# ushasigh/srsran-edgeric-5g

Hardware: AMD Instinct MI355X
Metric: pdsch_slots_per_sec (higher is better)
Workload: dtype u32 bit-packed GF(2) + bf16 grid + f32 IQ

## Files before the change

### srsran-edgeric-5g_amd/build.py

```python
import os
import subprocess
import sys

HERE = os.path.dirname(os.path.abspath(__file__))
ROOT = os.path.dirname(HERE)
CSRC = os.path.join(HERE, "csrc")
LIB = os.path.join(CSRC, "libmi355nrphy.so")
SOURCES = ["nrphy_host.cpp", "pdsch_plan_build.cpp", "pdsch_host.cpp", "dl_control_host.cpp", "pdsch_async.cpp", "dl_slot_async.cpp",
           "ofdm_host.cpp", "lower_phy_host.cpp", "demod_host.cpp", "ldpc_dematcher_host.cpp", "ldpc_decoder_host.cpp", "pusch_decoder_host.cpp",
           "csi_rs_host.cpp", "pdsch_kernels.hip", "ofdm_kernels.hip", "ldpc_decoder.hip",
           "ldpc_dematcher.hip", "pusch_decoder.hip", "csi_rs_kernels.hip", "dl_control_kernels.hip", "lower_phy_kernels.hip", "demod_kernels.hip",
           "pusch_demod_host.cpp", "pusch_demod_kernels.hip", "pusch_chest_host.cpp", "pusch_chest_kernels.hip",
           "prach_host.cpp", "prach_kernels.hip", "prach_demod_host.cpp", "prach_demod_kernels.hip", "pucch_host.cpp", "pucch_kernels.hip",
           "pucch2_host.cpp", "pucch2_kernels.hip", "srs_host.cpp", "srs_kernels.hip",
           "uci_host.cpp", "uci_kernels.hip", "ulsch_host.cpp", "ulsch_kernels.hip", "ofh_ul_host.cpp", "ofh_ul_kernels.hip",
           "ofh_dl_host.cpp", "ofh_dl_kernels.hip", "ofh_rx_host.cpp", "ofh_rx_kernels.hip"]
HEADERS = ["nrphy_internal.h", "nrphy_host_internal.h", "pdsch_plan.h", "pdsch_staging_host.h", "ldpc_receive_host.h", "ldpc_base_graph_host.h", "pusch_alloc_host.h", "ulsch_placement_host.h", "nrphy_trace.h", "bits_device.h", "crc24b_fold.h", "ofh_compress_device.h", "ofh_ul_chunk_device.h", "chest_device.h", "chest_host.h", "demod_device.h", "equalize_device.h", "ldpc_device.h", "fft_device.h", "nr_ldpc_bg.inc", "nr_polar_tables.inc", "prach_tables.inc", "prach_demod_tables.inc", "pucch_tables.inc", "srs_tables.inc", "uci_tables.inc",
           os.path.join(ROOT, "include", "mi355_nrphy.h")]
HIPCC = os.environ.get("HIPCC", "/opt/rocm/bin/hipcc")
MAX_COMPILERS = 16
CONTRACT = {}
FLAGS = ["--offload-arch=gfx950", "-O3", "-std=c++17", "-fPIC", "-Wall",
         "-I" + os.path.join(ROOT, "include"), "-I" + CSRC]


def _stale():
    if not os.path.exists(LIB):
        return True
    t = os.path.getmtime(LIB)
    deps = [os.path.join(CSRC, s) for s in SOURCES] + [h if os.path.isabs(h) else os.path.join(CSRC, h) for h in HEADERS]
    return any(os.path.getmtime(d) > t for d in deps)


def build(force=False, verbose=False):
    if not force and not _stale():
        return LIB
    objs = []
    cmds = []
    for src in SOURCES:
        obj = os.path.join(CSRC, os.path.splitext(src)[0] + ".o")
        cmds.append([HIPCC] + FLAGS + [CONTRACT.get(src, "-ffp-contract=off"), "-x", "hip", "-c", os.path.join(CSRC, src),
                     "-o", obj])
        objs.append(obj)
    procs = []
    try:
        while cmds or procs:
            while cmds and len(procs) < MAX_COMPILERS:
                cmd = cmds.pop(0)
                if verbose:
                    print(" ".join(cmd))
                procs.append((cmd, subprocess.Popen(cmd, stdout=subprocess.PIPE, stderr=subprocess.STDOUT)))
            cmd, p = procs.pop(0)
            out, _ = p.communicate(timeout=1800)
            if p.returncode != 0:
                raise RuntimeError("hipcc failed: %s\n%s" % (" ".join(cmd), out.decode(errors="replace")))
            if verbose and out:
                print(out.decode(errors="replace"))
    finally:
        for _, p in procs:
            p.kill()
    cmd = [HIPCC, "--offload-arch=gfx950", "-shared", "-fPIC", "-o", LIB] + objs
    subprocess.run(cmd, check=True, timeout=600)
    return LIB


if __name__ == "__main__":
    print(build(force="--force" in sys.argv, verbose=True))
```

### srsran-edgeric-5g_amd/csrc/nrphy_internal.h

```cpp
#pragma once

#include "mi355_nrphy.h"

#include <hip/hip_runtime.h>
#include <stdint.h>

namespace nrphy {

constexpr int NOF_LIFTING_SIZES = 51;
constexpr int NOF_GRAPHS        = 2 * NOF_LIFTING_SIZES;
constexpr int MAX_BG_ROWS       = 46;
constexpr int MAX_BG_EDGES      = 316;

struct LiftedGraph {
  uint16_t row_ptr[MAX_BG_ROWS + 2];
  uint16_t core_b;
  uint16_t core_s0;
  uint16_t core_s3;
  uint16_t core_mid;
  uint32_t edge[MAX_BG_EDGES];
};

#define NR_POLAR_SUBBLOCK_PATTERN                                                                                       \
  {0, 1, 2, 4, 3, 5, 6, 7, 8, 16, 9, 17, 10, 18, 11, 19, 12, 20, 13, 21, 14, 22, 15, 23, 24, 25, 26, 28, 27, 29, 30, 31}

constexpr int GOLD_JUMP_BITS  = 24;
constexpr int GOLD_X1_WORDS   = 1 << 16;

constexpr uint32_t SCR_PARTS = 4;

constexpr int CRC_POW_WORDS = 288;

struct GoldTables {
  uint32_t x2_jump[GOLD_JUMP_BITS][32];
  uint32_t x2_head[32][32];
  uint32_t crc24b_pow32[CRC_POW_WORDS];
  uint32_t crc24b_table[256];
  uint32_t crc24b_mul[CRC_POW_WORDS][6][16];
  float2 qam_lut[4][256];
};

constexpr int RE_CHUNK = 512;
#define NRPHY_CB_U_GRAPH_OFFSET (2 * 22 * 12 + 80)

enum SymKind : uint32_t { SYM_NONE = 0, SYM_CONTIGUOUS = 1, SYM_TABLE = 2 };

struct PduDev {
  uint64_t tb_offset;
  uint64_t cw_bit_offset;
  uint32_t tb_bytes;
  uint32_t grid_index;
  uint32_t graph;
  uint32_t zc;
  uint32_t kb;
  uint32_t K;
  uint32_t info_bits;
  uint32_t filler;
  uint32_t tb_crc_bits;
  uint32_t cb_crc_bits;
  uint32_t zero_pad;
  uint32_t C;
  uint32_t n_short;
  uint32_t e_short;
  uint32_t e_long;
  uint32_t n_cb;
  uint32_t k0;
  uint32_t nof_rows;
  uint32_t qm;
  uint32_t nof_layers;
  uint32_t nof_ports;
  uint32_t c_init;
  uint32_t item_first;
  uint32_t seed_first;
  uint32_t scr_words;
  uint32_t scr_word_offset;
  uint32_t nof_re;
  uint32_t weights_offset;
  uint32_t dmrs_weights_offset;
  uint32_t nof_prg;
  uint32_t prg_size_subc;
  uint32_t sym_re_start[NRPHY_NSYMB + 1];
  uint32_t sym_kind[NRPHY_NSYMB];
  uint32_t sym_arg[NRPHY_NSYMB];
  uint32_t dmrs_symbol_mask;
  uint32_t dmrs_zero_other_group;
  uint32_t dmrs_c_init[NRPHY_NSYMB];
  uint32_t dmrs_ref_rb;
  uint32_t dmrs_seq_offset;
  uint32_t dmrs_seq_words;
  float    dmrs_amplitude;
  uint32_t prb_mask[2 * NRPHY_PRB_WORDS];
  uint32_t first_prb;
  uint32_t end_prb;
  uint32_t crc_first;
  uint32_t crc_count;
};

struct CbWork {
  uint32_t pdu;
  uint32_t cb;
  uint32_t re_begin;
  uint32_t re_count;
};

constexpr int DMRS_PRB_CHUNK = 32;
#ifndef NRPHY_CRC_WORDS_PER_THREAD
#define NRPHY_CRC_WORDS_PER_THREAD 16
#endif
constexpr uint32_t TB_CRC_REGION_WORDS = 256 * NRPHY_CRC_WORDS_PER_THREAD;
constexpr uint32_t TB_CRC_REGION_BYTES = 4 * TB_CRC_REGION_WORDS;

struct TbCrcTables {
  uint32_t y32[2][4][256];
  uint32_t y1k[2][4][256];
  uint32_t y8k[2][4][256];
  uint32_t yz[2][4][256];
  uint32_t lane[2][64];
};

// ... 622 lines not shown
```

### srsran-edgeric-5g_amd/csrc/pdsch_kernels.hip

```cpp
#include "ldpc_device.h"

#ifndef NRPHY_PHASE_A_STAGED
#define NRPHY_PHASE_A_STAGED 1
#endif

#ifdef NRPHY_PROBES
#define NRPHY_STAGE(p) ((p).profile_stage)
#else
#define NRPHY_STAGE(p) 0u
#endif

namespace nrphy {

__global__ __launch_bounds__(TB_CRC_THREADS) void prologue_kernel(PdschLaunch p, const uint8_t* __restrict__ d_tb)
{
  constexpr uint32_t LDS_WORDS = TB_CRC_LDS_WORDS;
  __shared__ __attribute__((aligned(16))) uint32_t lds[LDS_WORDS];
  static_assert(LDS_WORDS >= GOLD_RING_WORDS, "LDS of the sequence role");
  const uint32_t tid = threadIdx.x;

  uint32_t scr_index = blockIdx.x, crc_index = blockIdx.x - p.n_scr_work;
  bool     scr_role  = blockIdx.x < p.n_scr_work;
  if (p.prologue_order == 1 && p.n_scr_work != 0 && p.n_crc_work != 0) {
    const uint32_t total = p.n_scr_work + p.n_crc_work;
    const uint32_t xcd = blockIdx.x & 7u, turn = blockIdx.x >> 3, q = total >> 3, r = total & 7u;
    const uint32_t pos = xcd * q + (xcd < r ? xcd : r) + turn;
    const uint32_t s0 = (uint32_t)(((uint64_t)pos * p.n_scr_work + total - 1u) / total);
    const uint32_t s1 = (uint32_t)(((uint64_t)(pos + 1u) * p.n_scr_work + total - 1u) / total);
    scr_role  = s1 > s0;
    scr_index = s0;
    crc_index = pos - s0;
  }
  NRPHY_WG_TRACE_MARK(0);
  NRPHY_WG_TRACE_WHERE(scr_role ? 1 : 2);
  if (scr_role) {
    if (NRPHY_STAGE(p) == 8) {
      return;
    }
    const auto*    swc   = to_constant(&p.scr_work[scr_index]);
    const uint32_t first = swc->first, count = swc->count;
    const bool     with_dmrs = swc->with_dmrs != 0;
    PduRef         pd    = *to_constant(&p.pdus[swc->pdu]);
    const uint32_t wave = tid / WAVE, lane = tid % WAVE;
    constexpr uint32_t DMRS_WAVES = TB_CRC_THREADS / WAVE - 1, DMRS_SCRATCH = (GOLD_RING_WORDS - 2048u) / DMRS_WAVES;
    static_assert(GOLD_SEED_WORDS <= 2048u && GOLD_RING_WORDS > 2048u, "LDS of the sequence role");
    static_assert((12u * NRPHY_MAX_RB + 31u) / 32u + 1u <= DMRS_SCRATCH, "DM-RS scratch per wave");
    if (wave == 0) {
      if (count == 0) {
        return;
      }
      if (p.scr_as_words != 0) {
        constexpr uint32_t SCR_STORE_ROWS = 8;
        uint32_t*       out = p.scr_seq + pd.scr_word_offset + first;
        const uint32_t* x1  = p.x1_words + first;
        gold_sequence_blocks_wave(p.gold, pd.c_init, first, count, lds, lane, [&](uint32_t base, uint32_t avail) {
          for (uint32_t k0 = lane; k0 < avail; k0 += SCR_STORE_ROWS * WAVE) {
            uint32_t x[SCR_STORE_ROWS];
// ... 230 lines not shown
    const uint32_t pad = (32u - (n & 31u)) & 31u;
    const uint32_t nw  = (n + pad) >> 5;
    const uint32_t per = (nw + WAVE - 1) / WAVE;
    uint32_t       a   = lane * per;
    uint32_t       b   = a + per;
    a                  = a > nw ? nw : a;
    b                  = b > nw ? nw : b;
    constexpr uint32_t CRC_MAX_PER = (22u * 384u / 32u + WAVE - 1u) / WAVE;
    const uint32_t     first = b - per, skip = a - first;
    uint32_t           word[CRC_MAX_PER];
    if (pad == 0) {
#pragma unroll
      for (uint32_t i = 0; i != CRC_MAX_PER; ++i) {
        word[i] = 0;
        if (i < per && i >= skip) {
          word[i] = sh->lin[first + i];
        }
      }
    } else {
#pragma unroll
      for (uint32_t i = 0; i != CRC_MAX_PER; ++i) {
        const uint32_t j = first + i;
        word[i]          = 0;
        if (i < per && i >= skip) {
          word[i] = (j == 0) ? sh->lin[0] >> pad : ext32(sh->lin, 32u * j - pad);
        }
      }
    }
    uint32_t res = 0, parity = 0;
#pragma unroll
    for (uint32_t i = 0; i != CRC_MAX_PER; ++i) {
      if (i < per) {
        res = crc24b_fold_word(res, word[i]);
        parity ^= word[i];
      }
    }
    const uint32_t reg = crc24b_fold_finish(res, parity);
    uint32_t part = 0;
    {
      const uint32_t m = nw - b;
#pragma unroll
      for (uint32_t k = 0; k != 6; ++k) {
        part ^= tables->crc24b_mul[m][k][(reg >> (4u * k)) & 15u];
      }
    }
    uint32_t crc = wave_xor(part);
    if (lane == 0) {
      or_bits_lds_exclusive(sh->lin, n, crc << 8, 24);
    }
    wave_sync();
  }
}

struct RmIndex {
  uint32_t fs;
  uint32_t flen;
  uint32_t n_valid;
  uint32_t rank0;
  float    inv_valid;
};

__device__ __forceinline__ RmIndex rm_index_init(PduRef pd)
{
  RmIndex  r;
  uint32_t nsys = (pd.kb - 2u) * pd.zc;
  uint32_t fs   = nsys - pd.filler;
  uint32_t fe   = nsys;
  fs            = fs > pd.n_cb ? pd.n_cb : fs;
  fe            = fe > pd.n_cb ? pd.n_cb : fe;
  r.fs          = fs;
  r.flen        = fe - fs;
  r.n_valid     = pd.n_cb - r.flen;
  r.rank0       = pd.k0 < fs ? pd.k0 : (pd.k0 < fe ? fs : pd.k0 - r.flen);
  r.inv_valid   = 1.0f / (float)r.n_valid;
  return r;
}

template <bool WRAP>
__device__ __forceinline__ uint32_t rm_gather32(const RmIndex& r, const uint32_t* lin, uint32_t zc2, uint32_t t)
{
  uint32_t u = r.rank0 + t;
  if (WRAP && u >= r.n_valid) {
    uint32_t q = (uint32_t)((float)u * r.inv_valid);
    u -= q * r.n_valid;
    if ((int32_t)u < 0) {
      u += r.n_valid;
    } else if (u >= r.n_valid) {
      u -= r.n_valid;
    }
  }
  uint32_t run = (u < r.fs) ? r.fs - u : r.n_valid - u;
  uint32_t out = ext32(lin, (u < r.fs ? u : u + r.flen) + zc2);
  if (run >= 32u) {
    return out;
  }
  out &= topmask(run);
  uint32_t filled = run;
  while (filled < 32u) {
    u += run;
    if (u >= r.n_valid) {
      if (!WRAP) {
        break;
      }
      u = 0;
    }
    run            = (u < r.fs) ? r.fs - u : r.n_valid - u;
    run            = run > 32u - filled ? 32u - filled : run;
    uint32_t piece = ext32(lin, (u < r.fs ? u : u + r.flen) + zc2);
    out |= (piece & topmask(run)) >> filled;
    filled += run;
  }
  return out;
}

__device__ __forceinline__ uint32_t bit_select(uint32_t m, uint32_t a, uint32_t b)
{
  return __builtin_amdgcn_bitop3_b32(m, a, b, 0xCA);
}

__device__ __forceinline__ void transpose8x8(uint32_t& hi, uint32_t& lo)
{
  hi = bit_select(0xAA55AA55u, hi, bit_select(0x55005500u, hi << 7, hi >> 7));
  lo = bit_select(0xAA55AA55u, lo, bit_select(0x55005500u, lo << 7, lo >> 7));
  hi = bit_select(0xCCCC3333u, hi, bit_select(0x33330000u, hi << 14, hi >> 14));
  lo = bit_select(0xCCCC3333u, lo, bit_select(0x33330000u, lo << 14, lo >> 14));
  const uint32_t nhi = bit_select(0xF0F0F0F0u, hi, lo >> 4);
  const uint32_t nlo = bit_select(0x0F0F0F0Fu, lo, hi << 4);
  hi                 = nhi;
  lo                 = nlo;
}

__device__ __forceinline__ void cmul_ref(float xr, float xi, float wr, float wi, float& outr, float& outi)
{
  float t0 = __fmul_rn(xi, wi);
  float t1 = __fmul_rn(xr, wi);
  outr     = __fmaf_rn(xr, wr, -t0);
  outi     = __fmaf_rn(xi, wr, t1);
}

typedef float cf2 __attribute__((ext_vector_type(2)));
__device__ __forceinline__ cf2 cmul_ref_packed(cf2 x, cf2 w)
{
  cf2 t, r;
  asm("v_pk_mul_f32 %0, %1, %2 op_sel:[1,1] op_sel_hi:[0,1]" : "=v"(t) : "v"(x), "v"(w));
  asm("v_pk_fma_f32 %0, %1, %2, %3 op_sel_hi:[1,0,1] neg_lo:[0,0,1]" : "=v"(r) : "v"(x), "v"(w), "v"(t));
  return r;
}
__device__ __forceinline__ cf2 cmul_ref_packed_uniform(cf2 x, cf2 w)
{
  cf2 t, r;
  asm("v_pk_mul_f32 %0, %1, %2 op_sel:[1,1] op_sel_hi:[0,1]" : "=v"(t) : "v"(x), "s"(w));
  asm("v_pk_fma_f32 %0, %1, %2, %3 op_sel_hi:[1,0,1] neg_lo:[0,0,1]" : "=v"(r) : "v"(x), "s"(w), "v"(t));
  return r;
}

typedef __bf16 bf16x2_t __attribute__((ext_vector_type(2)));
typedef float  f32x2_t __attribute__((ext_vector_type(2)));
__device__ __forceinline__ uint32_t pack_cbf16(float re, float im)
{
  f32x2_t  v = {re, im};
  bf16x2_t b = __builtin_convertvector(v, bf16x2_t);
  return *reinterpret_cast<uint32_t*>(&b);
}

__device__ __forceinline__ void grid_store(uint32_t* p, uint32_t v)
{
  __builtin_nontemporal_store(v, p);
}

#ifndef NRPHY_GRID_STORE_AUX
#define NRPHY_GRID_STORE_AUX 2
#endif
#ifndef NRPHY_GRID_BUFFER_STORES
#define NRPHY_GRID_BUFFER_STORES 1
#endif

struct ChunkGeom {
  uint32_t E;
  uint32_t cw_cb;
  uint32_t bit0;
};

template <int QM, int L, bool WRAP>
__device__ __forceinline__ void phase_a(const PdschLaunch& p, PduRef pd, const CbWork& wk, const CbShared& sh,
                                        uint32_t E, uint32_t lane)
{
  const uint32_t esym = E / QM;
  const uint32_t zc2  = 2u * pd.zc;
  const RmIndex  rm   = rm_index_init(pd);
  const uint32_t s0   = wk.re_begin * L;
  const uint32_t nblk = (wk.re_count * L + 31u) >> 5;
  constexpr uint32_t LUT_TRIPS = ((1u << QM) + WAVE - 1u) / WAVE;
  float2             lut[LUT_TRIPS];
#pragma unroll
  for (uint32_t k = 0; k != LUT_TRIPS; ++k) {
    lut[k] = lane + WAVE * k < (1u << QM) ? p.gold->qam_lut[QM / 2 - 1][lane + WAVE * k] : make_float2(0.f, 0.f);
  }
#if NRPHY_PHASE_A_STAGED
  for (uint32_t item = lane; item < QM * nblk; item += WAVE) {
    const uint32_t blk = item / QM, j = item - blk * QM;
    sh.symb[8u * blk + j] = rm_gather32<WRAP>(rm, sh.lin, zc2, j * esym + s0 + 32u * blk);
  }
  wave_sync();
  const uint8_t* rows = reinterpret_cast<const uint8_t*>(sh.symb);
  for (uint32_t item = lane; item < 4u * nblk; item += WAVE) {
    const uint32_t blk = item >> 2, m = item & 3u;
    const uint8_t* b   = rows + 32u * blk + (3u - m);
    uint32_t       r8[8];
#pragma unroll
    for (int j = 0; j != 8; ++j) {
      r8[j] = (j < QM) ? b[4 * j] : 0u;
    }
    uint32_t hi = (r8[0] << 24) | (r8[1] << 16) | (r8[2] << 8) | r8[3];
    uint32_t lo = (r8[4] << 24) | (r8[5] << 16) | (r8[6] << 8) | r8[7];
    transpose8x8(hi, lo);
    sh.symb[8u * blk + 2u * m]      = hi;
    sh.symb[8u * blk + 2u * m + 1u] = lo;
  }
#else
  for (uint32_t blk = lane; blk < nblk; blk += WAVE) {
    uint32_t row[8];
#pragma unroll
    for (int j = 0; j != 8; ++j) {
      row[j] = (j < QM) ? rm_gather32<WRAP>(rm, sh.lin, zc2, (uint32_t)j * esym + s0 + 32u * blk) : 0u;
    }
#pragma unroll
    for (int m = 0; m != 4; ++m) {
      const int sft = 24 - 8 * m;
      uint32_t  hi  = (((row[0] >> sft) & 0xFFu) << 24) | (((row[1] >> sft) & 0xFFu) << 16) |
                    (((row[2] >> sft) & 0xFFu) << 8) | ((row[3] >> sft) & 0xFFu);
      uint32_t lo = (((row[4] >> sft) & 0xFFu) << 24) | (((row[5] >> sft) & 0xFFu) << 16) |
                    (((row[6] >> sft) & 0xFFu) << 8) | ((row[7] >> sft) & 0xFFu);
      transpose8x8(hi, lo);
      sh.symb[8u * blk + 2u * m]      = hi;
      sh.symb[8u * blk + 2u * m + 1u] = lo;
    }
  }
#endif
  if (lane < 8) {
    sh.symb[8u * nblk + lane] = 0;
  }
#pragma unroll
  for (uint32_t k = 0; k != LUT_TRIPS; ++k) {
    if (lane + WAVE * k < (1u << QM)) {
      reinterpret_cast<float2*>(sh.u)[lane + WAVE * k] = lut[k];
    }
  }
  wave_sync();
}

__device__ __forceinline__ void pin_scalar(cf2& w)
{
  asm volatile("" : "+s"(w));
}

struct ChunkMap {
  uint32_t re0;
  uint32_t word0;
  bool     aligned;
  const uint32_t* gwords;
};

template <int QM, int L>
__device__ __forceinline__ uint32_t global_bits(const ChunkGeom& g, const ChunkMap& cm, uint32_t re_count, uint32_t r)
{
  uint32_t bits = 0;
  if (r < re_count) {
    if (QM * L == 32 && cm.aligned) {
      bits = (cm.gwords + cm.word0)[r];
    } else {
      bits = ext32(cm.gwords, g.bit0 + r * (uint32_t)(QM * L));
    }
  }
  return bits;
}
template <int QM, int L>
__device__ __forceinline__ uint32_t x2_bits(const uint32_t* x2, const ChunkGeom& g, const ChunkMap& cm, uint32_t r)
{
  if (QM * L == 32 && cm.aligned) {
    return x2[r];
  }
  return ext32(x2, (g.bit0 & 31u) + r * (uint32_t)(QM * L));
}

template <int QM, int L, bool WORDS>
__device__ __forceinline__ void re_bits(const CbShared& sh, const ChunkGeom& g, const ChunkMap& cm,
                                        uint32_t re_count, uint32_t r, uint32_t& bytes, uint32_t& gbits)
{
  if constexpr (L == 4) {
    bytes = sh.symb[r];
  } else {
// ... 150 lines not shown
      for (int l = 0; l != L; ++l) {
        const uint32_t raw = ((bytes >> (24 - 8 * l)) & 0xFFu) >> (8 - QM);
        v_rm |= raw << (32 - (l + 1) * QM);
      }
      if (d_cw_rm) {
        or_bits_global(d_cw_rm, cw_bit0 + (uint64_t)r * LQ, v_rm, LQ);
      }
      if (d_cw_scr) {
        or_bits_global(d_cw_scr, cw_bit0 + (uint64_t)r * LQ, v_rm ^ (gbits & topmask(LQ)), LQ);
      }
    }
  }
  if (d_grid == nullptr) {
    return;
  }
  const uint32_t nof_ports = pd.nof_prg == 1 ? pd.nof_ports : 0u;
  if (nof_ports == 4u) {
    phase_b_grid<QM, L, 4, WORDS>(p, pd, pd_global, wk, sh, g, cm, first_gbits, lane, d_grid);
  } else if (L <= 3 && nof_ports == 3u) {
    phase_b_grid<QM, (L <= 3 ? L : 1), 3, WORDS>(p, pd, pd_global, wk, sh, g, cm, first_gbits, lane, d_grid);
  } else if (L <= 2 && nof_ports == 2u) {
    phase_b_grid<QM, (L <= 2 ? L : 1), 2, WORDS>(p, pd, pd_global, wk, sh, g, cm, first_gbits, lane, d_grid);
  } else if (L == 1 && nof_ports == 1u) {
    phase_b_grid<QM, 1, 1, WORDS>(p, pd, pd_global, wk, sh, g, cm, first_gbits, lane, d_grid);
  } else {
    phase_b_grid<QM, L, 0, WORDS>(p, pd, pd_global, wk, sh, g, cm, first_gbits, lane, d_grid);
  }
}

template <int QM, int L, bool WORDS>
__device__ __forceinline__ void map_chunk(const PdschLaunch& p, PduRef pd, const PduDev* pd_global, const CbWork& wk,
                                          uint32_t item, const CbShared& sh, uint32_t lane, uint32_t* d_grid,
                                          uint32_t* d_cw_rm, uint32_t* d_cw_scr)
{
  const bool is_long = wk.cb >= pd.n_short;
  ChunkGeom  g;
  g.E     = is_long ? pd.e_long : pd.e_short;
  g.cw_cb = is_long ? pd.n_short * pd.e_short + (wk.cb - pd.n_short) * pd.e_long : wk.cb * pd.e_short;
  g.bit0  = g.cw_cb + wk.re_begin * (uint32_t)(QM * L);
  if (NRPHY_STAGE(p) == 3) {
    return;
  }
  ChunkMap cm;
  cm.re0     = g.cw_cb / (uint32_t)(QM * L) + wk.re_begin;
  cm.word0   = g.bit0 >> 5;
  cm.aligned = (g.bit0 & 31u) == 0;
  cm.gwords  = WORDS ? p.scr_seq + pd.scr_word_offset : p.x1_words;
  uint32_t seed_word = 0u;
  if constexpr (!WORDS) {
    const uint32_t seed_slot = pd.seed_first + (item - pd.item_first);
    seed_word                = lane < 31u ? p.scr_seq[(size_t)seed_slot * 32u + lane] : 0u;
  }
  const uint32_t first_gbits = global_bits<QM, L>(g, cm, wk.re_count, lane);
  {
    const RmIndex rm = rm_index_init(pd);
    if (rm.rank0 + g.E > rm.n_valid) {
      phase_a<QM, L, true>(p, pd, wk, sh, g.E, lane);
    } else {
      phase_a<QM, L, false>(p, pd, wk, sh, g.E, lane);
    }
  }
  if (NRPHY_STAGE(p) == 4) {
    return;
  }
  NRPHY_WG_TRACE_MARK(3);
  if constexpr (!WORDS) {
    static_assert((31u + (uint32_t)RE_CHUNK * 32u + 31u) / 32u + 1u <= GOLD_EXPAND_MAX_WORDS, "a work item's scrambling words");
    gold_expand_seed_wave(sh.lin, seed_word, ((g.bit0 & 31u) + wk.re_count * (uint32_t)(QM * L) + 31u) / 32u + 1u, lane);
  }
  phase_b<QM, L, WORDS>(p, pd, pd_global, wk, sh, g, cm, first_gbits, lane, d_grid, d_cw_rm, d_cw_scr);
}

template <int QM, bool WORDS>
__device__ __forceinline__ void map_chunk_layers(const PdschLaunch& p, PduRef pd, const PduDev* pd_global,
                                                 const CbWork& wk, uint32_t item, const CbShared& sh, uint32_t lane,
                                                 uint32_t* d_grid, uint32_t* d_cw_rm, uint32_t* d_cw_scr)
{
  switch (pd.nof_layers) {
    case 1:
      map_chunk<QM, 1, WORDS>(p, pd, pd_global, wk, item, sh, lane, d_grid, d_cw_rm, d_cw_scr);
      break;
    case 2:
      map_chunk<QM, 2, WORDS>(p, pd, pd_global, wk, item, sh, lane, d_grid, d_cw_rm, d_cw_scr);
      break;
    case 3:
      map_chunk<QM, 3, WORDS>(p, pd, pd_global, wk, item, sh, lane, d_grid, d_cw_rm, d_cw_scr);
      break;
    default:
      map_chunk<QM, 4, WORDS>(p, pd, pd_global, wk, item, sh, lane, d_grid, d_cw_rm, d_cw_scr);
      break;
  }
}

template <int L, typename W>
__device__ __forceinline__ void dmrs_port_words(float dr, float di, bool odd, uint32_t port, W w, uint32_t (&word)[(L + 1) / 2])
{
  const float sr = odd ? -dr : dr, si = odd ? -di : di;
#pragma unroll
  for (int g = 0; g != (L + 1) / 2; ++g) {
    float accr, acci;
    cmul_ref(dr, di, w[2 * (port * L + 2 * g)], w[2 * (port * L + 2 * g) + 1], accr, acci);
    if (2 * g + 1 < L) {
      float pr, pi;
      cmul_ref(sr, si, w[2 * (port * L + 2 * g + 1)], w[2 * (port * L + 2 * g + 1) + 1], pr, pi);
      accr = __fadd_rn(accr, pr);
      acci = __fadd_rn(acci, pi);
    }
    word[g] = pack_cbf16(accr, acci);
  }
}

typedef uint32_t u32x2_t __attribute__((ext_vector_type(2)));
typedef uint32_t u32x4_t __attribute__((ext_vector_type(4)));
// ... 477 lines not shown
```

### srsran-edgeric-5g_amd/csrc/pdsch_plan_build.cpp

```cpp
#include "pdsch_plan.h"

#include <algorithm>
#include <array>
#include <cmath>
#include <cstring>
#include <map>
#include <new>
#include <unordered_map>
#include <vector>

namespace {

struct SeqKey {
  std::array<uint32_t, 6>               scr;
  std::array<uint32_t, 2 + NRPHY_NSYMB> dmrs;
  bool operator==(const SeqKey& o) const { return scr == o.scr && dmrs == o.dmrs; }
};
struct SeqKeyHash {
  size_t operator()(const SeqKey& k) const
  {
    uint64_t h = 0xCBF29CE484222325ULL;
    for (uint32_t w : k.scr) {
      h = (h ^ w) * 0x100000001B3ULL;
    }
// ... 460 lines not shown
    copy_mapping(pd, cached->second);
    return pd.sym_re_start[NRPHY_NSYMB];
  }
  PlanShapeCache::Remap        built;
  const PlanShapeCache::Remap* rel = nullptr;
  if (shapes != nullptr) {
    auto known = shapes->remap.find(remap_sig);
    if (known != shapes->remap.end()) {
      rel = &known->second;
    }
  }
  if (rel == nullptr) {
    build_remap(pdus[i], built);
    rel = &built;
    if (shapes != nullptr) {
      rel = &shapes->remap.insert({remap_sig, built}).first->second;
    }
  }
  const uint32_t base = (uint32_t)t.re_table.size();
  t.re_table.insert(t.re_table.end(), rel->table.begin(), rel->table.end());
  ReMapping m;
  copy_mapping(m, rel->m);
  for (unsigned l = 0; l != NRPHY_NSYMB; ++l) {
    m.sym_arg[l] += (m.sym_kind[l] == SYM_TABLE ? base : 0U);
  }
  copy_mapping(pd, m);
  remap_cache.insert({remap_sig, m});
  return pd.sym_re_start[NRPHY_NSYMB];
}

void PlanBuilder::describe_pdu(uint32_t i, const nrphy_pdsch_derived_t& d, PduDev& pd)
{
  const nrphy_pdsch_pdu_t& pdu = pdus[i];
  const unsigned           kb  = (pdu.ldpc_base_graph == 1) ? 22 : 10;
  pd.tb_offset      = tb_offset[i];
  pd.cw_bit_offset  = cw_bits;
  pd.tb_bytes       = pdu.tb_size_bytes;
  pd.grid_index     = grid_index ? grid_index[i] : 0;
  pd.graph          = (pdu.ldpc_base_graph - 1) * NOF_LIFTING_SIZES + (uint32_t)lifting_position(d.lifting_size);
  pd.zc             = d.lifting_size;
  pd.kb             = kb;
  pd.K              = d.segment_length;
  pd.info_bits      = d.cb_info_bits;
  pd.filler         = d.nof_filler_bits;
  pd.tb_crc_bits    = d.nof_tb_crc_bits;
  pd.cb_crc_bits    = d.nof_cb_crc_bits;
  pd.zero_pad       = d.zero_pad;
  pd.C              = d.nof_codeblocks;
  pd.n_short        = d.nof_short_segments;
  pd.e_short        = d.rm_length_short;
  pd.e_long         = d.rm_length_long;
  pd.n_cb           = d.n_cb;
  pd.k0             = d.k0;
  pd.qm             = pdu.qm;
  pd.nof_layers     = pdu.nof_layers;
  pd.nof_ports      = pdu.nof_ports;
  pd.c_init         = (pdu.rnti << 15) + pdu.n_id;
  pd.nof_re         = d.nof_re;
  {
    const unsigned nsys = (kb - 2) * d.lifting_size;
    unsigned       fs = std::min(nsys - d.nof_filler_bits, d.n_cb), fe = std::min(nsys, d.n_cb);
    const unsigned flen = fe - fs, n_valid = d.n_cb - flen;
    const unsigned rank0 = d.k0 < fs ? d.k0 : (d.k0 < fe ? fs : d.k0 - flen);
    unsigned       last;
    if (rank0 + d.rm_length_long > n_valid) {
      last = d.n_cb - 1;
    } else {
      unsigned u = rank0 + d.rm_length_long - 1;
      last       = u < fs ? u : u + flen;
    }
    const unsigned nodes = divide_ceil(last + 1 + 2 * d.lifting_size, d.lifting_size);
    pd.nof_rows          = std::max(4U, nodes > kb ? nodes - kb : 0U);
  }
  {
    const float avg     = (pdu.qm == 2) ? 2.0F : (pdu.qm == 4) ? 10.0F : (pdu.qm == 6) ? 42.0F : 170.0F;
    float       scaling = std::sqrt(1 / avg);
    const float cfg     = std::pow(10.0F, -pdu.ratio_pdsch_data_to_sss_dB / 20.0F);
    if (std::isnormal(cfg)) {
      scaling *= cfg;
    }
    const unsigned nw      = 2 * pdu.nof_prg * pdu.nof_ports * pdu.nof_layers;
    pd.weights_offset      = (uint32_t)t.weights.size();
    for (unsigned k = 0; k != nw; ++k) {
      t.weights.push_back(pdu.precoding ? pdu.precoding[k] * scaling : 0.0F);
    }
    pd.dmrs_weights_offset = (uint32_t)t.weights.size();
    for (unsigned k = 0; k != nw; ++k) {
      t.weights.push_back(pdu.precoding ? pdu.precoding[k] : 0.0F);
    }
    pd.nof_prg       = pdu.nof_prg;
    pd.prg_size_subc = pdu.prg_size_rb * 12;
  }
  pd.dmrs_symbol_mask = pdu.dmrs_symbol_mask;
  pd.dmrs_zero_other_group = (pdu.nof_cdm_groups_without_data == 2 && (pdu.nof_layers + 1) / 2 == 1) ? 1U : 0U;
  pd.dmrs_ref_rb      = (pdu.ref_point == 1) ? pdu.bwp_start_rb : 0;
  {
    const float amp   = std::pow(10.0F, -pdu.ratio_pdsch_dmrs_to_sss_dB / 20.0F);
    pd.dmrs_amplitude = (float)(M_SQRT1_2 * (double)amp);
  }
  for (unsigned l = 0; l != NRPHY_NSYMB; ++l) {
    const uint64_t a  = (uint64_t)(14 * pdu.slot_index + l + 1) * (2 * pdu.scrambling_id + 1);
    pd.dmrs_c_init[l] = (uint32_t)(((a << 17) + (2 * pdu.scrambling_id + (pdu.n_scid ? 1 : 0))) & 0x7FFFFFFFULL);
    if ((pdu.dmrs_symbol_mask >> l) & 1U) {
      const uint32_t first = (uint32_t)mask_lowest(pdu.prb_mask), end = (uint32_t)mask_highest(pdu.prb_mask) + 1;
      for (uint32_t b = first; b < end; b += DMRS_PRB_CHUNK) {
        t.dmrs.push_back({i, l, b, std::min<uint32_t>(end, b + DMRS_PRB_CHUNK)});
      }
    }
  }
  for (unsigned w = 0; w != NRPHY_PRB_WORDS; ++w) {
    pd.prb_mask[2 * w]     = (uint32_t)pdu.prb_mask[w];
    pd.prb_mask[2 * w + 1] = (uint32_t)(pdu.prb_mask[w] >> 32);
  }
  pd.first_prb = (uint32_t)mask_lowest(pdu.prb_mask);
  pd.end_prb   = (uint32_t)mask_highest(pdu.prb_mask) + 1;
  if (pdu.nof_cdm_groups_without_data < (pdu.nof_layers + 1) / 2) {
    plan.dmrs_separate = true;
  }
  pdus_of_grid[pd.grid_index].push_back(i);
  pd.scr_words = (d.codeword_bits + 31U) / 32U + 1U + 31U;
  pd.dmrs_seq_words = (12U * (pd.end_prb - pd.dmrs_ref_rb) + 31U) / 32U + 1U;
}
// ... 282 lines not shown
```

Before: 1.306 million.

## Restructure rate-match gather and bit interleave into one-lane-per-block register transpose

Replaces the two-pass staged rate-matching gather and 8x8 transpose in phase_a with a single pass in which each lane owns one 32-RE block. In the common non-wrapping case it reads each row with an unaligned word pair plus alignbit, patches filler-gap crossings separately, and transposes in registers with delta swaps and byte permutes before storing with vector writes. The rate-match index is now precomputed on the host and stored in the PDU struct. This removes a wave sync, LDS round-trips and per-bit run loops, but adds a larger PDU struct and divergent fallback paths for wrapping or gap-crossing rows.

```diff
diff --git a/srsran-edgeric-5g_amd/build.py b/srsran-edgeric-5g_amd/build.py
--- a/srsran-edgeric-5g_amd/build.py
+++ b/srsran-edgeric-5g_amd/build.py
@@ -15,7 +15,7 @@
            "pucch2_host.cpp", "pucch2_kernels.hip", "srs_host.cpp", "srs_kernels.hip",
            "uci_host.cpp", "uci_kernels.hip", "ulsch_host.cpp", "ulsch_kernels.hip", "ofh_ul_host.cpp", "ofh_ul_kernels.hip",
            "ofh_dl_host.cpp", "ofh_dl_kernels.hip", "ofh_rx_host.cpp", "ofh_rx_kernels.hip"]
-HEADERS = ["nrphy_internal.h", "nrphy_host_internal.h", "pdsch_plan.h", "pdsch_staging_host.h", "ldpc_receive_host.h", "ldpc_base_graph_host.h", "pusch_alloc_host.h", "ulsch_placement_host.h", "nrphy_trace.h", "bits_device.h", "crc24b_fold.h", "ofh_compress_device.h", "ofh_ul_chunk_device.h", "chest_device.h", "chest_host.h", "demod_device.h", "equalize_device.h", "ldpc_device.h", "fft_device.h", "nr_ldpc_bg.inc", "nr_polar_tables.inc", "prach_tables.inc", "prach_demod_tables.inc", "pucch_tables.inc", "srs_tables.inc", "uci_tables.inc",
+HEADERS = ["nrphy_internal.h", "nrphy_host_internal.h", "pdsch_plan.h", "pdsch_staging_host.h", "ldpc_receive_host.h", "ldpc_base_graph_host.h", "pusch_alloc_host.h", "ulsch_placement_host.h", "nrphy_trace.h", "bits_device.h", "crc24b_fold.h", "rm_interleave.h", "ofh_compress_device.h", "ofh_ul_chunk_device.h", "chest_device.h", "chest_host.h", "demod_device.h", "equalize_device.h", "ldpc_device.h", "fft_device.h", "nr_ldpc_bg.inc", "nr_polar_tables.inc", "prach_tables.inc", "prach_demod_tables.inc", "pucch_tables.inc", "srs_tables.inc", "uci_tables.inc",
            os.path.join(ROOT, "include", "mi355_nrphy.h")]
 HIPCC = os.environ.get("HIPCC", "/opt/rocm/bin/hipcc")
 MAX_COMPILERS = 16
diff --git a/srsran-edgeric-5g_amd/csrc/nrphy_internal.h b/srsran-edgeric-5g_amd/csrc/nrphy_internal.h
--- a/srsran-edgeric-5g_amd/csrc/nrphy_internal.h
+++ b/srsran-edgeric-5g_amd/csrc/nrphy_internal.h
@@ -1,6 +1,7 @@
 #pragma once
 
 #include "mi355_nrphy.h"
+#include "rm_interleave.h"
 
 #include <hip/hip_runtime.h>
 #include <stdint.h>
@@ -65,6 +66,7 @@
   uint32_t e_long;
   uint32_t n_cb;
   uint32_t k0;
+  RmIndex  rm;
   uint32_t nof_rows;
   uint32_t qm;
   uint32_t nof_layers;
diff --git a/srsran-edgeric-5g_amd/csrc/pdsch_kernels.hip b/srsran-edgeric-5g_amd/csrc/pdsch_kernels.hip
--- a/srsran-edgeric-5g_amd/csrc/pdsch_kernels.hip
+++ b/srsran-edgeric-5g_amd/csrc/pdsch_kernels.hip
@@ -1,8 +1,4 @@
 #include "ldpc_device.h"
-
-#ifndef NRPHY_PHASE_A_STAGED
-#define NRPHY_PHASE_A_STAGED 1
-#endif
 
 #ifdef NRPHY_PROBES
 #define NRPHY_STAGE(p) ((p).profile_stage)
@@ -339,82 +335,9 @@
   }
 }
 
-struct RmIndex {
-  uint32_t fs;
-  uint32_t flen;
-  uint32_t n_valid;
-  uint32_t rank0;
-  float    inv_valid;
-};
-
-__device__ __forceinline__ RmIndex rm_index_init(PduRef pd)
-{
-  RmIndex  r;
-  uint32_t nsys = (pd.kb - 2u) * pd.zc;
-  uint32_t fs   = nsys - pd.filler;
-  uint32_t fe   = nsys;
-  fs            = fs > pd.n_cb ? pd.n_cb : fs;
-  fe            = fe > pd.n_cb ? pd.n_cb : fe;
-  r.fs          = fs;
-  r.flen        = fe - fs;
-  r.n_valid     = pd.n_cb - r.flen;
-  r.rank0       = pd.k0 < fs ? pd.k0 : (pd.k0 < fe ? fs : pd.k0 - r.flen);
-  r.inv_valid   = 1.0f / (float)r.n_valid;
-  return r;
-}
-
-template <bool WRAP>
-__device__ __forceinline__ uint32_t rm_gather32(const RmIndex& r, const uint32_t* lin, uint32_t zc2, uint32_t t)
-{
-  uint32_t u = r.rank0 + t;
-  if (WRAP && u >= r.n_valid) {
-    uint32_t q = (uint32_t)((float)u * r.inv_valid);
-    u -= q * r.n_valid;
-    if ((int32_t)u < 0) {
-      u += r.n_valid;
-    } else if (u >= r.n_valid) {
-      u -= r.n_valid;
-    }
-  }
-  uint32_t run = (u < r.fs) ? r.fs - u : r.n_valid - u;
-  uint32_t out = ext32(lin, (u < r.fs ? u : u + r.flen) + zc2);
-  if (run >= 32u) {
-    return out;
-  }
-  out &= topmask(run);
-  uint32_t filled = run;
-  while (filled < 32u) {
-    u += run;
-    if (u >= r.n_valid) {
-      if (!WRAP) {
-        break;
-      }
-      u = 0;
-    }
-    run            = (u < r.fs) ? r.fs - u : r.n_valid - u;
-    run            = run > 32u - filled ? 32u - filled : run;
-    uint32_t piece = ext32(lin, (u < r.fs ? u : u + r.flen) + zc2);
-    out |= (piece & topmask(run)) >> filled;
-    filled += run;
-  }
-  return out;
-}
-
-__device__ __forceinline__ uint32_t bit_select(uint32_t m, uint32_t a, uint32_t b)
-{
-  return __builtin_amdgcn_bitop3_b32(m, a, b, 0xCA);
-}
-
-__device__ __forceinline__ void transpose8x8(uint32_t& hi, uint32_t& lo)
-{
-  hi = bit_select(0xAA55AA55u, hi, bit_select(0x55005500u, hi << 7, hi >> 7));
-  lo = bit_select(0xAA55AA55u, lo, bit_select(0x55005500u, lo << 7, lo >> 7));
-  hi = bit_select(0xCCCC3333u, hi, bit_select(0x33330000u, hi << 14, hi >> 14));
-  lo = bit_select(0xCCCC3333u, lo, bit_select(0x33330000u, lo << 14, lo >> 14));
-  const uint32_t nhi = bit_select(0xF0F0F0F0u, hi, lo >> 4);
-  const uint32_t nlo = bit_select(0x0F0F0F0Fu, lo, hi << 4);
-  hi                 = nhi;
-  lo                 = nlo;
+__device__ __forceinline__ RmIndex rm_index_of(PduRef pd)
+{
+  return {pd.rm.fs, pd.rm.flen, pd.rm.n_valid, pd.rm.rank0, pd.rm.inv_valid};
 }
 
 __device__ __forceinline__ void cmul_ref(float xr, float xi, float wr, float wi, float& outr, float& outi)
@@ -474,7 +397,7 @@
 {
   const uint32_t esym = E / QM;
   const uint32_t zc2  = 2u * pd.zc;
-  const RmIndex  rm   = rm_index_init(pd);
+  const RmIndex  rm   = rm_index_of(pd);
   const uint32_t s0   = wk.re_begin * L;
   const uint32_t nblk = (wk.re_count * L + 31u) >> 5;
   constexpr uint32_t LUT_TRIPS = ((1u << QM) + WAVE - 1u) / WAVE;
@@ -483,47 +406,75 @@
   for (uint32_t k = 0; k != LUT_TRIPS; ++k) {
     lut[k] = lane + WAVE * k < (1u << QM) ? p.gold->qam_lut[QM / 2 - 1][lane + WAVE * k] : make_float2(0.f, 0.f);
   }
-#if NRPHY_PHASE_A_STAGED
-  for (uint32_t item = lane; item < QM * nblk; item += WAVE) {
-    const uint32_t blk = item / QM, j = item - blk * QM;
-    sh.symb[8u * blk + j] = rm_gather32<WRAP>(rm, sh.lin, zc2, j * esym + s0 + 32u * blk);
-  }
-  wave_sync();
-  const uint8_t* rows = reinterpret_cast<const uint8_t*>(sh.symb);
-  for (uint32_t item = lane; item < 4u * nblk; item += WAVE) {
-    const uint32_t blk = item >> 2, m = item & 3u;
-    const uint8_t* b   = rows + 32u * blk + (3u - m);
-    uint32_t       r8[8];
-#pragma unroll
-    for (int j = 0; j != 8; ++j) {
-      r8[j] = (j < QM) ? b[4 * j] : 0u;
-    }
-    uint32_t hi = (r8[0] << 24) | (r8[1] << 16) | (r8[2] << 8) | r8[3];
-    uint32_t lo = (r8[4] << 24) | (r8[5] << 16) | (r8[6] << 8) | r8[7];
-    transpose8x8(hi, lo);
-    sh.symb[8u * blk + 2u * m]      = hi;
-    sh.symb[8u * blk + 2u * m + 1u] = lo;
-  }
-#else
-  for (uint32_t blk = lane; blk < nblk; blk += WAVE) {
-    uint32_t row[8];
-#pragma unroll
-    for (int j = 0; j != 8; ++j) {
-      row[j] = (j < QM) ? rm_gather32<WRAP>(rm, sh.lin, zc2, (uint32_t)j * esym + s0 + 32u * blk) : 0u;
-    }
-#pragma unroll
-    for (int m = 0; m != 4; ++m) {
-      const int sft = 24 - 8 * m;
-      uint32_t  hi  = (((row[0] >> sft) & 0xFFu) << 24) | (((row[1] >> sft) & 0xFFu) << 16) |
-                    (((row[2] >> sft) & 0xFFu) << 8) | ((row[3] >> sft) & 0xFFu);
-      uint32_t lo = (((row[4] >> sft) & 0xFFu) << 24) | (((row[5] >> sft) & 0xFFu) << 16) |
-                    (((row[6] >> sft) & 0xFFu) << 8) | ((row[7] >> sft) & 0xFFu);
-      transpose8x8(hi, lo);
-      sh.symb[8u * blk + 2u * m]      = hi;
-      sh.symb[8u * blk + 2u * m + 1u] = lo;
-    }
-  }
-#endif
+  static_assert((uint32_t)RE_CHUNK * L / 32u <= WAVE && CB_U_QAM_WORDS % 4u == 0, "a lane per block; aligned blocks");
+  if (lane < nblk) {
+    const auto      ext     = [&](uint32_t pos) { return ext32(sh.lin, pos); };
+    uint32_t        w[8]    = {};
+    uint32_t        general = 0;
+    const uint32_t  u0      = rm.rank0 + s0;
+    if (!WRAP && u0 + (uint32_t)(QM - 1) * esym + 32u * nblk <= rm.n_valid) {
+      u32x2_unaligned pair[QM];
+      uint32_t        shift[QM];
+      uint32_t        meets = 0;
+#pragma unroll
+      for (int j = 0; j != QM; ++j) {
+        const uint32_t    u    = u0 + (uint32_t)j * esym;
+        const uint32_t    side = rm_gap_side(u, 32u * nblk, rm.fs);
+        const RmClearRead rd   = rm_clear_read(u + (side == RM_ABOVE ? rm.flen : 0u) + zc2);
+        meets |= (side == RM_MEETS ? 1u : 0u) << j;
+        pair[j]  = *reinterpret_cast<const u32x2_unaligned*>(sh.lin + (rd.word + lane));
+        shift[j] = rd.shift;
+      }
+#pragma unroll
+      for (int j = 0; j != QM; ++j) {
+        w[j] = rm_clear_word(pair[j].x, pair[j].y, shift[j]);
+      }
+#pragma unroll 1
+      while (meets != 0) {
+        const uint32_t j = (uint32_t)__builtin_ctz(meets);
+        meets &= meets - 1u;
+        const uint32_t        u  = u0 + j * esym;
+        const RmClearRead     ra = rm_clear_read(u + rm.flen + zc2);
+        const u32x2_unaligned v  = *reinterpret_cast<const u32x2_unaligned*>(sh.lin + (ra.word + lane));
+        const uint32_t        above = rm_clear_word(v.x, v.y, ra.shift);
+        const uint32_t        keep  = rm_gap_mask(u + 32u * lane, rm.fs);
+#pragma unroll
+        for (uint32_t k = 0; k != QM; ++k) {
+          w[k] = bit_select(keep | (k == j ? 0u : 0xFFFFFFFFu), w[k], above);
+        }
+      }
+    } else {
+      u32x2_unaligned pair[QM];
+      uint32_t        shift[QM];
+#pragma unroll
+      for (int j = 0; j != QM; ++j) {
+        const RmRow       row = rm_row<WRAP>(rm, zc2, (uint32_t)j * esym + s0, 32u * nblk);
+        const RmClearRead rd  = rm_clear_read(row.pos);
+        const uint32_t    own = row.clear ? 1u : 0u;
+        general |= (own ^ 1u) << j;
+        pair[j]  = *reinterpret_cast<const u32x2_unaligned*>(sh.lin + (rd.word + __umul24(lane, own)));
+        shift[j] = rd.shift;
+      }
+#pragma unroll
+      for (int j = 0; j != QM; ++j) {
+        w[j] = rm_clear_word(pair[j].x, pair[j].y, shift[j]);
+      }
+#pragma unroll 1
+      while (general != 0) {
+        const uint32_t j = (uint32_t)__builtin_ctz(general);
+        general &= general - 1u;
+        const uint32_t g = rm_gather32<WRAP>(rm, ext, zc2, j * esym + s0 + 32u * lane);
+#pragma unroll
+        for (uint32_t k = 0; k != QM; ++k) {
+          w[k] = k == j ? g : w[k];
+        }
+      }
+    }
+    rm_transpose_block<QM>(w);
+    uint4* out = reinterpret_cast<uint4*>(sh.symb + 8u * lane);
+    out[0]     = make_uint4(w[0], w[1], w[2], w[3]);
+    out[1]     = make_uint4(w[4], w[5], w[6], w[7]);
+  }
   if (lane < 8) {
     sh.symb[8u * nblk + lane] = 0;
   }
@@ -780,13 +731,10 @@
     seed_word                = lane < 31u ? p.scr_seq[(size_t)seed_slot * 32u + lane] : 0u;
   }
   const uint32_t first_gbits = global_bits<QM, L>(g, cm, wk.re_count, lane);
-  {
-    const RmIndex rm = rm_index_init(pd);
-    if (rm.rank0 + g.E > rm.n_valid) {
-      phase_a<QM, L, true>(p, pd, wk, sh, g.E, lane);
-    } else {
-      phase_a<QM, L, false>(p, pd, wk, sh, g.E, lane);
-    }
+  if (pd.rm.rank0 + g.E > pd.rm.n_valid) {
+    phase_a<QM, L, true>(p, pd, wk, sh, g.E, lane);
+  } else {
+    phase_a<QM, L, false>(p, pd, wk, sh, g.E, lane);
   }
   if (NRPHY_STAGE(p) == 4) {
     return;
diff --git a/srsran-edgeric-5g_amd/csrc/pdsch_plan_build.cpp b/srsran-edgeric-5g_amd/csrc/pdsch_plan_build.cpp
--- a/srsran-edgeric-5g_amd/csrc/pdsch_plan_build.cpp
+++ b/srsran-edgeric-5g_amd/csrc/pdsch_plan_build.cpp
@@ -536,22 +536,19 @@
   pd.e_long         = d.rm_length_long;
   pd.n_cb           = d.n_cb;
   pd.k0             = d.k0;
+  pd.rm             = rm_index(kb, d.lifting_size, d.nof_filler_bits, d.n_cb, d.k0);
   pd.qm             = pdu.qm;
   pd.nof_layers     = pdu.nof_layers;
   pd.nof_ports      = pdu.nof_ports;
   pd.c_init         = (pdu.rnti << 15) + pdu.n_id;
   pd.nof_re         = d.nof_re;
   {
-    const unsigned nsys = (kb - 2) * d.lifting_size;
-    unsigned       fs = std::min(nsys - d.nof_filler_bits, d.n_cb), fe = std::min(nsys, d.n_cb);
-    const unsigned flen = fe - fs, n_valid = d.n_cb - flen;
-    const unsigned rank0 = d.k0 < fs ? d.k0 : (d.k0 < fe ? fs : d.k0 - flen);
-    unsigned       last;
-    if (rank0 + d.rm_length_long > n_valid) {
+    unsigned last;
+    if (pd.rm.rank0 + d.rm_length_long > pd.rm.n_valid) {
       last = d.n_cb - 1;
     } else {
-      unsigned u = rank0 + d.rm_length_long - 1;
-      last       = u < fs ? u : u + flen;
+      unsigned u = pd.rm.rank0 + d.rm_length_long - 1;
+      last       = u < pd.rm.fs ? u : u + pd.rm.flen;
     }
     const unsigned nodes = divide_ceil(last + 1 + 2 * d.lifting_size, d.lifting_size);
     pd.nof_rows          = std::max(4U, nodes > kb ? nodes - kb : 0U);
diff --git a/srsran-edgeric-5g_amd/csrc/rm_interleave.h b/srsran-edgeric-5g_amd/csrc/rm_interleave.h
--- /dev/null
+++ b/srsran-edgeric-5g_amd/csrc/rm_interleave.h
@@ -0,0 +1,216 @@
+#pragma once
+
+#include <stdint.h>
+
+#ifndef NRPHY_HD
+#if defined(__HIPCC__)
+#define NRPHY_HD __attribute__((host)) __attribute__((device)) inline __attribute__((always_inline))
+#else
+#define NRPHY_HD inline
+#endif
+#endif
+
+namespace nrphy {
+
+struct RmIndex {
+  uint32_t fs;
+  uint32_t flen;
+  uint32_t n_valid;
+  uint32_t rank0;
+  float    inv_valid;
+};
+
+NRPHY_HD RmIndex rm_index(uint32_t kb, uint32_t zc, uint32_t filler, uint32_t n_cb, uint32_t k0)
+{
+  RmIndex  r;
+  uint32_t nsys = (kb - 2u) * zc;
+  uint32_t fs   = nsys - filler;
+  uint32_t fe   = nsys;
+  fs            = fs > n_cb ? n_cb : fs;
+  fe            = fe > n_cb ? n_cb : fe;
+  r.fs          = fs;
+  r.flen        = fe - fs;
+  r.n_valid     = n_cb - r.flen;
+  r.rank0       = k0 < fs ? k0 : (k0 < fe ? fs : k0 - r.flen);
+  r.inv_valid   = 1.0f / (float)r.n_valid;
+  return r;
+}
+
+NRPHY_HD uint32_t rm_reduce(const RmIndex& r, uint32_t u)
+{
+  const uint32_t q = (uint32_t)((float)u * r.inv_valid);
+  u -= q * r.n_valid;
+  if ((int32_t)u < 0) {
+    u += r.n_valid;
+  } else if (u >= r.n_valid) {
+    u -= r.n_valid;
+  }
+  return u;
+}
+
+NRPHY_HD uint32_t rm_topmask(uint32_t n)
+{
+  return n == 0 ? 0u : (0xFFFFFFFFu << (32u - n));
+}
+
+template <bool WRAP, class Ext32>
+NRPHY_HD uint32_t rm_gather32(const RmIndex& r, Ext32&& ext, uint32_t zc2, uint32_t t)
+{
+  uint32_t u = r.rank0 + t;
+  if (WRAP && u >= r.n_valid) {
+    u = rm_reduce(r, u);
+  }
+  uint32_t run = (u < r.fs) ? r.fs - u : r.n_valid - u;
+  uint32_t out = ext((u < r.fs ? u : u + r.flen) + zc2);
+  if (run >= 32u) {
+    return out;
+  }
+  out &= rm_topmask(run);
+  uint32_t filled = run;
+  while (filled < 32u) {
+    u += run;
+    if (u >= r.n_valid) {
+      if (!WRAP) {
+        break;
+      }
+      u = 0;
+    }
+    run            = (u < r.fs) ? r.fs - u : r.n_valid - u;
+    run            = run > 32u - filled ? 32u - filled : run;
+    uint32_t piece = ext((u < r.fs ? u : u + r.flen) + zc2);
+    out |= (piece & rm_topmask(run)) >> filled;
+    filled += run;
+  }
+  return out;
+}
+
+struct RmRow {
+  bool     clear;
+  uint32_t pos;
+};
+
+template <bool WRAP>
+NRPHY_HD RmRow rm_row(const RmIndex& r, uint32_t zc2, uint32_t t0, uint32_t span)
+{
+  uint32_t u = r.rank0 + t0;
+  if (WRAP && u >= r.n_valid) {
+    u = rm_reduce(r, u);
+  }
+  const uint32_t end   = u + span;
+  const bool     below = end <= r.fs;
+  RmRow          row;
+  row.clear = below || ((u >= r.fs || r.flen == 0u) && end <= r.n_valid);
+  row.pos   = (below ? u : u + r.flen) + zc2;
+  return row;
+}
+
+struct RmClearRead {
+  uint32_t word;
+  uint32_t shift;
+};
+NRPHY_HD RmClearRead rm_clear_read(uint32_t pos)
+{
+  return {(pos - 1u) >> 5, 31u - ((pos - 1u) & 31u)};
+}
+NRPHY_HD uint32_t rm_clear_word(uint32_t first, uint32_t second, uint32_t shift)
+{
+#if defined(__HIP_DEVICE_COMPILE__)
+  return __builtin_amdgcn_alignbit(first, second, shift);
+#else
+  return (uint32_t)((((uint64_t)first << 32) | second) >> shift);
+#endif
+}
+
+NRPHY_HD uint32_t bit_select(uint32_t m, uint32_t a, uint32_t b)
+{
+#if defined(__HIP_DEVICE_COMPILE__)
+  return __builtin_amdgcn_bitop3_b32(m, a, b, 0xCA);
+#else
+  return (a & m) | (b & ~m);
+#endif
+}
+
+enum RmGapSide : uint32_t { RM_BELOW = 0, RM_ABOVE = 1, RM_MEETS = 2 };
+NRPHY_HD uint32_t rm_gap_side(uint32_t u, uint32_t span, uint32_t fs)
+{
+  return u >= fs ? RM_ABOVE : (u + span <= fs ? RM_BELOW : RM_MEETS);
+}
+NRPHY_HD uint32_t rm_gap_mask(uint32_t u, uint32_t fs)
+{
+  const int32_t  d = (int32_t)(fs - u);
+  const uint32_t k = d < 0 ? 0u : (d > 32 ? 32u : (uint32_t)d);
+  return rm_topmask(k);
+}
+NRPHY_HD uint32_t rm_gap_word(uint32_t below, uint32_t above, uint32_t u, uint32_t fs)
+{
+  return bit_select(rm_gap_mask(u, fs), below, above);
+}
+
+NRPHY_HD uint32_t byte_perm(uint32_t hi, uint32_t lo, uint32_t sel)
+{
+#if defined(__HIP_DEVICE_COMPILE__)
+  return __builtin_amdgcn_perm(hi, lo, sel);
+#else
+  const uint64_t v = ((uint64_t)hi << 32) | lo;
+  uint32_t       out = 0;
+  for (int i = 0; i != 4; ++i) {
+    out |= (uint32_t)((v >> (8u * ((sel >> (8 * i)) & 7u))) & 0xFFu) << (8 * i);
+  }
+  return out;
+#endif
+}
+
+template <uint32_t KEEP, uint32_t SHIFT, bool B_ZERO>
+NRPHY_HD void rm_delta_swap(uint32_t& a, uint32_t& b)
+{
+  if (B_ZERO) {
+    b = (a & ~KEEP) << SHIFT;
+    a = a & KEEP;
+  } else {
+    const uint32_t na = bit_select(KEEP, a, b >> SHIFT);
+    b                 = bit_select(~KEEP, b, a << SHIFT);
+    a                 = na;
+  }
+}
+
+NRPHY_HD void rm_transpose_bytes4(uint32_t a, uint32_t b, uint32_t c, uint32_t d, uint32_t& w3, uint32_t& w2, uint32_t& w1,
+                                  uint32_t& w0)
+{
+  const uint32_t ab_hi = byte_perm(a, b, 0x07030602u), ab_lo = byte_perm(a, b, 0x05010400u);
+  const uint32_t cd_hi = byte_perm(c, d, 0x07030602u), cd_lo = byte_perm(c, d, 0x05010400u);
+  w3 = byte_perm(ab_hi, cd_hi, 0x07060302u);
+  w2 = byte_perm(ab_hi, cd_hi, 0x05040100u);
+  w1 = byte_perm(ab_lo, cd_lo, 0x07060302u);
+  w0 = byte_perm(ab_lo, cd_lo, 0x05040100u);
+}
+
+template <int QM>
+NRPHY_HD void rm_transpose_block(uint32_t (&w)[8])
+{
+  static_assert(QM == 2 || QM == 4 || QM == 6 || QM == 8, "modulation order");
+  for (int j = QM; j < 8; ++j) {
+    w[j] = 0u;
+  }
+  rm_delta_swap<0xF0F0F0F0u, 4, (QM <= 4)>(w[0], w[4]);
+  rm_delta_swap<0xF0F0F0F0u, 4, (QM <= 4)>(w[1], w[5]);
+  if (QM > 2) {
+    rm_delta_swap<0xF0F0F0F0u, 4, (QM <= 6)>(w[2], w[6]);
+    rm_delta_swap<0xF0F0F0F0u, 4, (QM <= 6)>(w[3], w[7]);
+  }
+  rm_delta_swap<0xCCCCCCCCu, 2, (QM == 2)>(w[0], w[2]);
+  rm_delta_swap<0xCCCCCCCCu, 2, (QM == 2)>(w[1], w[3]);
+  rm_delta_swap<0xCCCCCCCCu, 2, (QM == 2)>(w[4], w[6]);
+  rm_delta_swap<0xCCCCCCCCu, 2, (QM == 2)>(w[5], w[7]);
+  rm_delta_swap<0xAAAAAAAAu, 1, false>(w[0], w[1]);
+  rm_delta_swap<0xAAAAAAAAu, 1, false>(w[2], w[3]);
+  rm_delta_swap<0xAAAAAAAAu, 1, false>(w[4], w[5]);
+  rm_delta_swap<0xAAAAAAAAu, 1, false>(w[6], w[7]);
+  uint32_t q[8];
+  rm_transpose_bytes4(w[0], w[1], w[2], w[3], q[0], q[2], q[4], q[6]);
+  rm_transpose_bytes4(w[4], w[5], w[6], w[7], q[1], q[3], q[5], q[7]);
+  for (int k = 0; k != 8; ++k) {
+    w[k] = q[k];
+  }
+}
+
+}
```

New measurement: 1.300 million. About the same (-0.4%).
